# carlostojal/NDT-Net

Hardware: AMD Instinct MI355X
Metric: clouds/sec NDT preprocess+PointNet fwd, 100k pts->1000 NDs, batch=16 (higher is better)
Workload: dtype f64 NDT; PointNet fp32-accurate split-bf16x3 (6 products) on 11 per-point layers, fp32 MFMA on the K=16 first layers and the TNet / seg-bias FC layers

## Files before the change

### include/ndnet_pointnet.h

```cpp
#ifndef NDNET_POINTNET_H_
#define NDNET_POINTNET_H_
#include <stdint.h>

#ifdef __cplusplus
extern "C" {
#endif

#define NDNET_PN_MAX_LAYERS 5

typedef struct ndnet_pn_layer {
  const float* w;
  int64_t w_cloud_stride;
  const float* bias;
  int64_t bias_cloud_stride;
  int32_t K, N;
  int32_t relu;
  int32_t prec;
  int32_t fuse_next;
} ndnet_pn_layer;

typedef struct ndnet_pn_chain {
  const float* x;
  int32_t x_ld;
  int32_t in_cols;
// ... 14 lines not shown
  const float* head_w3;
  const float* head_b3;
  const float* head_basis;
  int32_t head_kin, head_nout;
  float* head_t1;
  const float* fold_t2;
  int32_t fold_ld;
  float* fold_out_w;
  float* fold_out_b;
} ndnet_pn_chain;

int ndnet_pn_chain_run(const ndnet_pn_chain *args, int batch, void *stream);
int ndnet_pn_chain_run_t32(const ndnet_pn_chain *args, int batch, void *stream);

int ndnet_pn_debug_stamps(unsigned long long *host, int wgs);
int ndnet_pn_debug_stamps_clear(void);

int ndnet_pn_fc_run(const float *in, int ld_in, const float *W, const float *bias, float *out, int ld_out,
                    int batch, int K, int N, int relu, void *stream);
int ndnet_pn_fc_mfma_run(const float *in, int ld_in, const float *Wf, const float *bias, float *out, int ld_out,
                         int batch, int K, int N, int relu, void *stream);
int ndnet_pn_cls_head_run(const float *in, int ld_in, const float *Wf, const float *bias, float *probs,
                          int ld_probs, float *logits, int ld_logits, int batch, int K, int N, int out_cols,
                          float *clear, int64_t clear_count, void *stream);
#define NDNET_FOLD_WT 0
#define NDNET_FOLD_FRAG 1
#define NDNET_FOLD_FRAG6 2
#define NDNET_FOLD_ROWS 3
#define NDNET_FOLD_BASIS 4
#define NDNET_FOLD_BIAS 5
typedef struct ndnet_pn_fold_job {
  const float *w;
  const float *bias;
  const float *gamma, *beta, *mean, *var;
  void *out;
  int32_t kind;
  int32_t N, K;
  int32_t ld, k0;
  int32_t Kp, Np;
  int32_t eye;
  float eps;
  int32_t reserved;
  int64_t block0;
} ndnet_pn_fold_job;
int ndnet_pn_fold_prepare(ndnet_pn_fold_job *host_jobs, int num_jobs, int64_t *num_blocks);
int ndnet_pn_fold_run(const ndnet_pn_fold_job *device_jobs, int num_jobs, int64_t num_blocks, void *stream);

int ndnet_pn_head3_run(const float *h2, int ld_h, const float *W3, const float *b3, const float *basis,
                       float *t1, float *w1f, int batch, int K, int kin, int nout, void *stream);

int ndnet_pn_fold_t2_run(const float *w1f, int w1_stride, const float *b1, const float *t2, int t2_ld, float *outf,
                         float *outb, int batch, void *stream);

#ifdef __cplusplus
}
#endif

#endif
```

### ndt-net_amd/csrc/pointnet_kernels.hip

```cpp
#include <hip/hip_runtime.h>
#include <math.h>
#include <stdint.h>
#include <stdio.h>
#include <stdlib.h>

#include "../../include/ndnet_pointnet.h"

namespace {

#ifndef NDNET_PN_TILE
#define NDNET_PN_TILE 64
#endif
constexpr int kP = NDNET_PN_TILE;
#ifndef NDNET_PN_WAVES
#define NDNET_PN_WAVES (NDNET_PN_TILE / 4)
#endif
constexpr int kWaves = NDNET_PN_WAVES;
constexpr int kThreads = 64 * kWaves;
constexpr int kRowBlocks = kP / 16;
static_assert(kP == 64 || kP == 32, "64- or 32-point tiles");
constexpr int kFuseNC = 64;
constexpr int kPadF = 8;
constexpr int kPadB = 16;
#ifndef NDNET_PN_PLANE_SWZ
// ... 1185 lines not shown
#pragma unroll
      for (int b = 0; b < 16; b++) v = lane == b ? acc[b] : v;
      s_part[wave][lane] = v;
    }
    __syncthreads();
    if (wq != 0) return;
    if (lane < 16) {
      float v = 0.0f;
#pragma unroll
      for (int q = 0; q < WPO; q++) v += s_part[wave + q][lane];
      acc[0] = v;
    }
  } else if (lane < 16) {
    float v = 0.0f;
#pragma unroll
    for (int b = 0; b < 16; b++) v = lane == b ? acc[b] : v;
    acc[0] = v;
  }
  if (lane < B && n < N) {
    float v = acc[0] + bias[n];
    if (relu) v = fmaxf(v, 0.0f);
    out[(int64_t)lane * ld_out + n] = v;
  }
}

__global__ void __launch_bounds__(1024) k_pn_fold_t2(const float* __restrict__ w1f, int w1_stride,
                                                     const float* __restrict__ b1, const float* __restrict__ t2,
                                                     int t2_ld, float* __restrict__ outf, float* __restrict__ outb) {
  const int b = blockIdx.x, e = threadIdx.x;
  __shared__ float s_w[13 * 64];
  __shared__ float s_t[64 * 64];
  {
    const float* wb = w1f + (int64_t)b * w1_stride;
    if (e < 16 * 64) {
      const int cb = e >> 8, ln = (e >> 2) & 63, k = 4 * (ln >> 4) + (e & 3), n = 16 * cb + (ln & 15);
      const float v = wb[e];
      if (k < 12) s_w[k * 64 + n] = v;
    }
    if (e < 64) s_w[12 * 64 + e] = b1[e];
    const f32x4* tb = reinterpret_cast<const f32x4*>(t2 + (int64_t)b * t2_ld);
    reinterpret_cast<f32x4*>(s_t)[e] = tb[e];
  }
  __syncthreads();
  if (e < 13 * 64) {
    const int r = e >> 6, n = e & 63;
    float acc = 0.0f;
#pragma unroll 16
    for (int i = 0; i < 64; i++) acc = fmaf(s_w[r * 64 + i], s_t[i * 64 + n], acc);
    if (r < 12) outf[(int64_t)b * 1024 + ((((n >> 4) * 64 + ((r >> 2) & 3) * 16 + (n & 15)) << 2) + (r & 3))] = acc;
    else outb[(int64_t)b * 64 + n] = acc;
  }
}

__global__ void __launch_bounds__(256) k_pn_head3(const float* __restrict__ h2, int ld_h, const float* __restrict__ W3,
                                                  const float* __restrict__ b3, const float* __restrict__ basis,
                                                  float* __restrict__ t1_out, float* __restrict__ w1f, int K, int kin,
                                                  int nout) {
  __shared__ float s_t[9];
  const int b = blockIdx.x;
  const int lane = threadIdx.x & 63, wave = threadIdx.x >> 6;
  const float* h = h2 + (int64_t)b * ld_h;
  for (int o = wave; o < 9; o += 4) {
    float acc = 0.0f;
    for (int k = lane; k < K; k += 64) acc += h[k] * W3[(int64_t)o * K + k];
    for (int off = 32; off > 0; off >>= 1) acc += __shfl_xor(acc, off, 64);
    if (lane == 0) {
      s_t[o] = acc + b3[o];
      t1_out[b * 9 + o] = acc + b3[o];
    }
  }
  const int M = kin * nout, total = 16 * nout;
  auto kn = [&](int e, int& k, int& n) {
    const int cb = e >> 8, ln = (e >> 2) & 63;
    k = 4 * (ln >> 4) + (e & 3);
    n = 16 * cb + (ln & 15);
  };
  constexpr int kE = 4;
  float bas[kE][9];
#pragma unroll
  for (int i = 0; i < kE; i++) {
    const int e = threadIdx.x + i * blockDim.x;
    int k, n;
    kn(e, k, n);
#pragma unroll
    for (int a = 0; a < 9; a++) bas[i][a] = (e < total && k < kin) ? basis[a * M + k * nout + n] : 0.0f;
  }
  __syncthreads();
#pragma unroll
  for (int i = 0; i < kE; i++) {
    const int e = threadIdx.x + i * blockDim.x;
    if (e < total) {
      float acc = 0.0f;
#pragma unroll
      for (int a = 0; a < 9; a++) acc += s_t[a] * bas[i][a];
      w1f[(int64_t)b * total + e] = acc;
    }
  }
  for (int e = threadIdx.x + kE * blockDim.x; e < total; e += blockDim.x) {
    int k, n;
    kn(e, k, n);
    float acc = 0.0f;
    if (k < kin) {
#pragma unroll
      for (int a = 0; a < 9; a++) acc += s_t[a] * basis[a * M + k * nout + n];
    }
    w1f[(int64_t)b * total + e] = acc;
// ... 135 lines not shown
  hipStream_t st = (hipStream_t)stream;
  if (cbw == 4)
    k_pn_fc_mfma<4><<<nb / 4, kFcWaves * 64, 0, st>>>(in, ld_in, wf, bias, out, ld_out, batch, KG, relu);
  else if (cbw == 2)
    k_pn_fc_mfma<2><<<nb / 2, kFcWaves * 64, 0, st>>>(in, ld_in, wf, bias, out, ld_out, batch, KG, relu);
  else
    k_pn_fc_mfma<1><<<nb, kFcWaves * 64, 0, st>>>(in, ld_in, wf, bias, out, ld_out, batch, KG, relu);
  return hipGetLastError() == hipSuccess ? 0 : -21;
}

int ndnet_pn_cls_head_run(const float* in, int ld_in, const float* Wf, const float* bias, float* probs, int ld_probs,
                          float* logits, int ld_logits, int batch, int K, int N, int out_cols, float* clear,
                          int64_t clear_count, void* stream) {
  if (!in || !Wf || !bias || !probs || batch <= 0 || K <= 0 || K % 16 || K > 16 * kClsMaxG || N <= 0 || N % 16 ||
      N > 1024 || out_cols < 1 || out_cols > N || ld_in % 4 || ld_in < K || ld_probs < out_cols ||
      (logits && ld_logits < out_cols) || ((uintptr_t)in | (uintptr_t)Wf) % 16 || clear_count < 0 ||
      (!clear && clear_count))
    return -20;
  k_pn_cls_head<<<(batch + 15) / 16, kClsWaves * 64, (size_t)16 * N * sizeof(float), (hipStream_t)stream>>>(
      in, ld_in, reinterpret_cast<const f32x4*>(Wf), bias, probs, ld_probs, logits, ld_logits, batch, K / 16, N,
      out_cols, clear, clear_count);
  return hipGetLastError() == hipSuccess ? 0 : -21;
}

int ndnet_pn_fc_run(const float* in, int ld_in, const float* W, const float* bias, float* out, int ld_out, int batch,
                    int K, int N, int relu, void* stream) {
  if (!in || !W || !bias || !out || batch <= 0 || batch > 16 || K <= 0 || K % 4 || N <= 0 || ld_in % 4 ||
      ld_in < K || ld_out < N || ((uintptr_t)in | (uintptr_t)W) % 16)
    return -20;
  hipStream_t st = (hipStream_t)stream;
  switch (K % 256 == 0 && K <= 1024 ? K / 256 : 0) {
    case 2: k_pn_fc_split<2><<<(N + 1) / 2, 256, 0, st>>>(in, ld_in, W, bias, out, ld_out, batch, N, relu); break;
    case 4: k_pn_fc_split<4><<<N, 256, 0, st>>>(in, ld_in, W, bias, out, ld_out, batch, N, relu); break;
    default: k_pn_fc<<<(N + 3) / 4, 256, 0, st>>>(in, ld_in, W, bias, out, ld_out, batch, K, N, relu);
  }
  return hipGetLastError() == hipSuccess ? 0 : -21;
}

int ndnet_pn_head3_run(const float* h2, int ld_h, const float* W3, const float* b3, const float* basis, float* t1,
                       float* w1f, int batch, int K, int kin, int nout, void* stream) {
  if (!h2 || !W3 || !b3 || !basis || !t1 || !w1f || batch <= 0 || K <= 0 || ld_h < K || kin <= 0 || kin > 16 ||
      nout <= 0 || nout % 16)
    return -20;
  k_pn_head3<<<batch, 256, 0, (hipStream_t)stream>>>(h2, ld_h, W3, b3, basis, t1, w1f, K, kin, nout);
  return hipGetLastError() == hipSuccess ? 0 : -21;
}

int ndnet_pn_fold_t2_run(const float* w1f, int w1_stride, const float* b1, const float* t2, int t2_ld, float* outf,
                         float* outb, int batch, void* stream) {
  if (!w1f || !b1 || !t2 || !outf || !outb || batch <= 0 || w1_stride < 1024 || t2_ld < 4096 || t2_ld % 4 ||
      (uintptr_t)t2 % 16)
    return -20;
  k_pn_fold_t2<<<batch, 1024, 0, (hipStream_t)stream>>>(w1f, w1_stride, b1, t2, t2_ld, outf, outb);
  return hipGetLastError() == hipSuccess ? 0 : -21;
}

int ndnet_pn_fold_prepare(ndnet_pn_fold_job* jobs, int num_jobs, int64_t* num_blocks) {
  if (!jobs || num_jobs <= 0 || !num_blocks) return -20;
  int64_t blocks = 0;
  for (int i = 0; i < num_jobs; i++) {
    ndnet_pn_fold_job& J = jobs[i];
    const bool bn = J.gamma != nullptr;
    if (!J.out || (uintptr_t)J.out % 16 || J.kind < NDNET_FOLD_WT || J.kind > NDNET_FOLD_BIAS || J.N <= 0 ||
        (bn && (!J.beta || !J.mean || !J.var || !(J.eps >= 0.0f))) || (!bn && (J.beta || J.mean || J.var)))
      return -20;
    if (J.kind == NDNET_FOLD_BIAS) {
      if (!J.bias || J.Np < J.N || J.eye < 0 || (J.eye > 0 && J.eye * J.eye != J.N)) return -20;
    } else {
      if (!J.w || J.K <= 0 || J.k0 < 0 || J.ld < J.k0 + J.K) return -20;
      if (J.kind == NDNET_FOLD_WT && (J.Kp < J.K || J.Np < J.N)) return -20;
      if (J.kind == NDNET_FOLD_FRAG && (J.Kp < J.K || J.Np < J.N || J.Kp % 16 || J.Np % 16)) return -20;
      if (J.kind == NDNET_FOLD_FRAG6 && (J.Kp < J.K || J.Np < J.N || J.Kp % 32 || J.Np % 16)) return -20;
      if (J.kind == NDNET_FOLD_BASIS && J.K != 12) return -20;
    }
    J.block0 = blocks;
    blocks += (fold_units(J) + kFoldThreads - 1) / kFoldThreads;
  }
  if (blocks <= 0 || blocks > 0x7fffffff) return -20;
  *num_blocks = blocks;
  return 0;
}

int ndnet_pn_fold_run(const ndnet_pn_fold_job* jobs, int num_jobs, int64_t num_blocks, void* stream) {
  if (!jobs || num_jobs <= 0 || num_blocks <= 0 || num_blocks > 0x7fffffff) return -20;
  k_pn_fold<<<(unsigned)num_blocks, kFoldThreads, 0, (hipStream_t)stream>>>(jobs, num_jobs);
  return hipGetLastError() == hipSuccess ? 0 : -21;
}


int ndnet_pn_debug_stamps_clear(void) {
#ifdef NDNET_PN_STAMPS
  static unsigned long long zeros[kStampWgs][16];
  return hipMemcpyToSymbol(HIP_SYMBOL(g_pn_stamps), zeros, sizeof(zeros)) == hipSuccess ? 0 : -21;
#else
  return -20;
#endif
}

int ndnet_pn_debug_stamps(unsigned long long* host, int wgs) {
#ifdef NDNET_PN_STAMPS
  if (!host || wgs <= 0 || wgs > kStampWgs) return -20;
  if (hipDeviceSynchronize() != hipSuccess) return -21;
  return hipMemcpyFromSymbol(host, HIP_SYMBOL(g_pn_stamps), (size_t)wgs * 16 * sizeof(unsigned long long)) ==
                 hipSuccess ? 0 : -21;
#else
  (void)host; (void)wgs;
// ... 118 lines not shown
```

### ndt-net_amd/ndnet/_lib.py

```python
from __future__ import annotations

import ctypes
import os

import torch

PKG = os.path.dirname(os.path.abspath(__file__))
ROOT = os.path.dirname(PKG)
LIB_PATH = os.environ.get("NDNET_AMD_LIB") or os.path.join(ROOT, "lib", "libndnet_amd.so")

NDNET_OK = 0
NDNET_ERR_ARG = -20
NDNET_ERR_HIP = -21
NDNET_ERR_SYNC = -22
POINT_FILL = {"none": 0, "nearest": 1}
SEG_CONF_LDS_MAX_COLS = 63
FPS_THREADS = 512
FPS_LDS_POINTS = {"float32": 12288, "float64": 6144}
FPS_REG_POINTS = {"float32": 100352, "float64": 49152}


class NdtStats(ctypes.Structure):
    _fields_ = [
        ("rc", ctypes.c_int32),
# ... 84 lines not shown
    "ndnet_fps_run": (_I, [_P, _I, _U64, _U64, _P, _P, _P, _P, _P]),
    "ndnet_fps_run_f64": (_I, [_P, _I, _U64, _U64, _P, _P, _P, _P, _P]),
    "ndnet_nearest_sample_run": (_I, [_P, _I, _U64, _P, _P, _U64, _P, _P, _P, _P]),
    "ndnet_pn_transform3_run": (_I, [_P, ctypes.c_int64, _P, _P, ctypes.c_int64, _I, _U64, _P]),
    "ndnet_aug_work_bytes": (ctypes.c_size_t, [_I, _U64]),
    "ndnet_aug_run": (_I, [_P, _P, _P, _P, _I, _U64, _P, _P, _P, _P, _P, _P, _P]),
    "ndnet_pts_unpack_i16": (_I, [_P, _P, _I, _U64, _P, _P, _P]),
    "ndnet_ndt_debug_dump": (_I, [_P, _I, _P, _P, _P, _P, _P, _P, _P, _P, _P, _P, _P, _P]),
    "ndnet_ndt_debug_set_epoch": (_I, [_P, ctypes.c_uint32]),
    "ndnet_ndt_debug_set_kl_fuse": (_I, [_P, _I]),
    "ndnet_ndt_debug_set_list_sort": (_I, [_P, _I]),
    "ndnet_ndt_debug_get_list_sort": (_I, [_P]),
    "ndnet_ndt_debug_kl_marks": (_I, [_P, _P]),
    "ndnet_ndt_debug_front_marks": (_I, [_P, _P]),
    "ndnet_ndt_debug_wq_marks": (_I, [_P, _P, ctypes.POINTER(ctypes.c_uint32)]),
    "ndnet_debug_lu_chain": (_I, [_P, ctypes.c_uint32, _I, _P, _P, _P, _P]),
    "ndnet_ndt_debug_front_wg_marks": (_I, [_P, _P, ctypes.POINTER(_I)]),
    "ndnet_ndt_set_timing": (_I, [_P, _I]),
    "ndnet_ndt_stage_ms": (_I, [_P, _P]),
    "ndnet_amd_version": (ctypes.c_char_p, []),
}


def lib() -> ctypes.CDLL:
    global _lib
    if _lib is None:
        if not os.path.exists(LIB_PATH):
            raise RuntimeError(f"{LIB_PATH} is missing: build it with `make -C {ROOT}` "
                               "(there is no CPU fallback)")
        _lib = ctypes.CDLL(LIB_PATH)
        for name, (res, args) in EXPORTS.items():
            fn = getattr(_lib, name)
            fn.restype = res
            fn.argtypes = args
        for name, (res, args) in {**POINTNET_EXPORTS, **TRAIN_EXPORTS}.items():
            fn = getattr(_lib, name)
            fn.restype = res
            fn.argtypes = args
    return _lib


POINTNET_EXPORTS: dict = {
    "ndnet_pn_chain_run": (_I, [_P, _I, _P]),
    "ndnet_pn_chain_run_t32": (_I, [_P, _I, _P]),
    "ndnet_pn_debug_stamps": (_I, [_P, _I]),
    "ndnet_pn_debug_stamps_clear": (_I, []),
    "ndnet_ply_count": (_I, [ctypes.c_char_p, _I, ctypes.POINTER(_U64)]),
    "ndnet_ply_read": (_I, [ctypes.c_char_p, _I, _I, _P, _P, _U64, ctypes.POINTER(_U64), _I]),
    "ndnet_pn_fc_run": (_I, [_P, _I, _P, _P, _P, _I, _I, _I, _I, _I, _P]),
    "ndnet_pn_fc_mfma_run": (_I, [_P, _I, _P, _P, _P, _I, _I, _I, _I, _I, _P]),
    "ndnet_pn_cls_head_run": (_I, [_P, _I, _P, _P, _P, _I, _P, _I, _I, _I, _I, _I, _P, ctypes.c_int64, _P]),
    "ndnet_pn_head3_run": (_I, [_P, _I, _P, _P, _P, _P, _P, _I, _I, _I, _I, _P]),
    "ndnet_pn_fold_t2_run": (_I, [_P, _I, _P, _P, _I, _P, _P, _I, _P]),
    "ndnet_pn_fold_prepare": (_I, [_P, _I, ctypes.POINTER(ctypes.c_int64)]),
    "ndnet_pn_fold_run": (_I, [_P, _I, ctypes.c_int64, _P]),
}


_I64 = ctypes.c_int64

TRAIN_EXPORTS: dict = {
    "ndnet_tr_gemm": (_I, [_P, _P, _P, _P, _I64, _I, _I, _I, _I64, _I64, _I64, _I64, _I64, _I64, _I, _I, _I, _I, _I,
                           _I, _P]),
    "ndnet_tr_sum_parts": (_I, [_P, _P, _I64, _I, _P]),
    "ndnet_tr_sum_parts_2d": (_I, [_P, _P, _I64, _I64, _I64, _I, _P]),
    "ndnet_tr_bn_fwd": (_I, [_P, _P, _P, _P, _P, _P, _P, _P, _I, _I, _I, ctypes.c_float, ctypes.c_float, _I, _P, _P,
                             _P, _P]),
    "ndnet_tr_bn_bwd": (_I, [_P, _P, _P, _P, _P, _P, _P, _P, _P, _P, _I, _I, _I, _I, _P, _P]),
    "ndnet_tr_chan_sum": (_I, [_P, _P, _I, _I, _I, _P]),
    "ndnet_tr_row_sum": (_I, [_P, _P, _I64, _I, _P]),
    "ndnet_tr_argmax_match": (_I, [_P, _P, _I64, _I, _P, _P]),
    "ndnet_tr_argmax_match_cm": (_I, [_P, _P, _I, _I, _I, _P, _P, _P]),
    "ndnet_row_argmax": (_I, [_P, _I64, _I, _P, _P]),
    "ndnet_tr_fc_fwd": (_I, [_P, _P, _P, _P, _P, _P, _P, _P, _P, _P, _P, _I, _I, _I, _I64, ctypes.c_float,
                             ctypes.c_float, _I, _I, _P, _P]),
    "ndnet_tr_fc_bwd_w": (_I, [_P, _P, _P, _P, _P, _P, _P, _P, _P, _P, _P, _P, _I, _I, _I, _I64, _I, _P]),
    "ndnet_tr_fc_bwd_x": (_I, [_P, _P, _P, _P, _I, _I, _I, _I64, _I, _P]),
    "ndnet_tr_point_transform": (_I, [_P, _P, _I, _P, _I, _P, _I, _I, _P]),
    "ndnet_tr_point_transform_bwd": (_I, [_P, _P, _I, _P, _I, _P, _I, _I, _P]),
    "ndnet_tr_log_softmax_c": (_I, [_P, _P, _I, _I, _I, _P]),
    "ndnet_tr_log_softmax_c_bwd": (_I, [_P, _P, _P, _I, _I, _I, _P]),
    "ndnet_tr_nll_onehot": (_I, [_P, _P, _P, _P, _I, _I, _I, _P]),
    "ndnet_tr_nll_onehot_bwd": (_I, [_P, _P, _P, _I, _I, _I, _P]),
    "ndnet_tr_nll_hist": (_I, [_P, _P, _P, _P, _P, _I, _I, _I, _P]),
    "ndnet_tr_nll_hist_bwd": (_I, [_P, _P, _P, _P, _I, _I, _I, _P]),
    "ndnet_tr_hist_match_cm": (_I, [_P, _P, _I, _I, _I, _P, _P, _P]),
    "ndnet_tr_adam": (_I, [_I, _P, _P, _P, _P, _P, _P, _P, ctypes.c_double, ctypes.c_double, ctypes.c_double,
                           ctypes.c_double, _P]),
}


def require_gpu() -> None:
    if not torch.cuda.is_available():
        raise RuntimeError("ndnet_amd needs a ROCm GPU (gfx950); none is visible and there is no CPU fallback")


def check(rc: int, what: str) -> None:
    if rc != NDNET_OK:
        raise RuntimeError(f"{what} failed with code {rc}")


def stream_ptr(device: torch.device | None = None) -> int:
    return torch.cuda.current_stream(device).cuda_stream
```

### ndt-net_amd/ndnet/models/pointnet_hip.py

```python
from __future__ import annotations

import ctypes
import os

import torch

from .. import _lib

MAX_LAYERS = 5
CHAIN_NAMES = ("A: TNet(3) 3-64-128-1024 + max", "B: conv1(t1) + TNet(64) 64-64-128-1024 + max",
               "C: conv1, conv2(t2), conv3 + max", "D: seg head 64-512-256-128-(C+1) + log_softmax")

chain_timing = None

MODES = {"x6": 1, "fp32": 1, "x3": 2, "bf16": 3}
PRECISION = SPLIT_BF16 = X6_PREC = None


def set_precision(mode: str) -> None:
    global PRECISION, SPLIT_BF16, X6_PREC
    if mode not in MODES:
        raise ValueError(f"unknown PointNet precision mode {mode!r}")
    PRECISION = mode
    SPLIT_BF16 = mode != "fp32"
# ... 373 lines not shown
def _use_t32(B: int, n: int, device) -> bool:
    if not TILE32:
        return False
    if device not in _cus:
        _cus[device] = torch.cuda.get_device_properties(device).multi_processor_count
    return 2 * B * ((n + 63) // 64) <= _cus[device]


def _run_chain(ch: "_Chain", x: torch.Tensor, out=None) -> None:
    assert x.stride(1) == ch.x_ld and x.stride(2) == 1 and x.dtype == torch.float32
    ch.x = x.data_ptr()
    ch.out = out.data_ptr() if out is not None else None
    if _use_t32(x.shape[0], x.shape[1], x.device):
        rc = _lib.lib().ndnet_pn_chain_run_t32(ctypes.byref(ch), x.shape[0], _lib.stream_ptr(x.device))
        _lib.check(rc, "ndnet_pn_chain_run_t32")
        return
    rc = _lib.lib().ndnet_pn_chain_run(ctypes.byref(ch), x.shape[0], _lib.stream_ptr(x.device))
    _lib.check(rc, "ndnet_pn_chain_run")


def _chain_torch(x: torch.Tensor, n: int, in_cols: int, layers, relus, mode: int, gmax=None, out=None,
                 out_cols=0, fuse=()) -> None:
    h = x[..., :in_cols].float()
    k0 = layers[0][0].shape[-2]
    h = torch.nn.functional.pad(h, (0, k0 - in_cols))
    for i, (w, b) in enumerate(layers):
        h = torch.matmul(h, w[..., : h.shape[-1], :]) + (b[:, None, :] if b.dim() == 2 else b)
        if relus[i]:
            h = torch.relu(h)
    if mode == 0:
        gmax.copy_(torch.maximum(gmax, h.amax(dim=1)))
    else:
        out.copy_(torch.log_softmax(h[..., :out_cols], dim=2))


class _Workspace:

    def __init__(self, W: _Folded, B: int, N: int, dev, mode: str = None) -> None:
        self.W = W
        self.mode = PRECISION if mode is None else mode
        f32 = dict(dtype=torch.float32, device=dev)
        Fp = W.C_tail[0].shape[1]
        self.gbuf = torch.full((B, 2048 + Fp), float("-inf"), **f32)
        self.g1, self.g2, self.g3 = self.gbuf[:, :1024], self.gbuf[:, 1024:2048], self.gbuf[:, 2048:]
        self.h1, self.h2 = torch.empty((B, 512), **f32), torch.empty((B, 256), **f32)
        self.t1, self.t2 = torch.empty((B, 9), **f32), torch.empty((B, 4096), **f32)
        self.cvec = torch.empty((B, 512), **f32)
        kin = 3 if W.baseline else 12
        self.w1T = None if W.baseline else torch.empty((B, 12, 64), **f32)
        self.w1t2 = torch.empty((B, kin, 64), **f32)
        self.b1t2 = torch.empty((B, 64), **f32)
        self.w1f = None if W.baseline else torch.empty((B, 16 * 64), **f32)
        self.w1t2f = torch.zeros((B, 16 * 64), **f32)
        if W.baseline:
            self.xt = torch.zeros((B, N, 4), **f32)
            self.pts = None
        first = (W.c1T16, W.c1b) if W.baseline else (self.w1T, W.c1b)
        self.specs = [
            (3, W.A, (1, 1, 1), 0, dict(gmax=self.g1)),
            (kin, [first] + W.B_tail, (0, 1, 1, 1), 0, dict(gmax=self.g2)),
            (kin, [(self.w1t2, self.b1t2), W.C_mid, W.C_tail], (0, 0, 0), 0, dict(gmax=self.g3)),
        ]
        if W.seg:
            self.specs.append((kin, [(self.w1t2, self.b1t2), (W.s1aT, self.cvec)] + W.D_tail, (0, 1, 1, 1, 0), 1,
                               dict(out_cols=W.C1, fuse=(1,))))
        self.N = N
        self.structs = {}

    def hip_layers(self, mode: str) -> list:
        W = self.W

        def shared(wb):
            w, b = wb
            if mode != "fp32" and id(w) in W.frag6:
                return (W.frag6[id(w)], 0, b, w.shape[0], w.shape[1], MODES[mode])
            return (W.frag[id(w)], 0, b, w.shape[0], w.shape[1])

        L1 = shared((W.c1T16, W.c1b)) if W.baseline else (self.w1f, self.w1f.stride(0), W.c1b, 16, 64)
        LC = (self.w1t2f, self.w1t2f.stride(0), self.b1t2, 16, 64) if FOLD_T2_KERNEL and not W.baseline else L1
        layers = [
            [shared(x) for x in W.A],
            [L1] + [shared(x) for x in W.B_tail],
            [LC, shared(W.C_mid), shared(W.C_tail)],
        ]
        if W.seg:
            layers.append([(self.w1t2f, self.w1t2f.stride(0), self.b1t2, 16, 64), shared((W.s1aT, self.cvec))] +
                          [shared(x) for x in W.D_tail])
        return layers

    def chain(self, i: int, x: torch.Tensor, chain_fn=None, out=None) -> None:
        in_cols, layers, relus, mode, kw = self.specs[i]
        if chain_fn is not None:
            kw = dict(kw)
            if out is not None:
                kw["out"] = out
            chain_fn(x, self.N, in_cols, layers, relus, mode, **kw)
            return
        structs = self.structs.get(self.mode)
        W = self.W
        if structs is None:
            x_lds = (3, 4, 4, 4) if W.baseline else (12, 12, 12, 12)
            structs = self.structs[self.mode] = [_build_chain(self.N, s[0], hl, s[2], s[3], x_ld=xl, **s[4])
                                                 for s, hl, xl in zip(self.specs, self.hip_layers(self.mode), x_lds)]
            if W.seg:
                structs[3].clear = self.gbuf.data_ptr()
                structs[3].clear_count = self.gbuf.numel()
            if HEAD3_IN_CHAIN and not W.baseline:
                cb = structs[1]
                cb.head_h2, cb.head_ld, cb.head_K = self.h2.data_ptr(), self.h2.stride(0), self.h2.shape[1]
                cb.head_w3, cb.head_b3 = W.t1["f3"].data_ptr(), W.t1["c3"].data_ptr()
                cb.head_basis, cb.head_kin, cb.head_nout = W.t1_basis.data_ptr(), 12, 64
                cb.head_t1 = self.t1.data_ptr()
            if not FOLD_T2_KERNEL or W.baseline:
                cc = structs[2]
                cc.fold_t2, cc.fold_ld = self.t2.data_ptr(), self.t2.stride(0)
                cc.fold_out_w, cc.fold_out_b = self.w1t2f.data_ptr(), self.b1t2.data_ptr()
        if chain_timing is not None:
            e0, e1 = torch.cuda.Event(enable_timing=True), torch.cuda.Event(enable_timing=True)
            e0.record()
            _run_chain(structs[i], x, out)
            e1.record()
            chain_timing.append((i, e0, e1))
        else:
            _run_chain(structs[i], x, out)


def _folded(model):
    cache = model._hip
    if cache is None:
        tensors = _tensors(model)
        cache = model._hip = {"tensors": tensors, "sig": None, "stale": False}
    sig = _signature(cache["tensors"])
    cur = _tensors(model)
    replaced = len(cur) != len(cache["tensors"]) or any(a is not b for a, b in zip(cur, cache["tensors"]))
    if replaced or cache["sig"] != sig or cache["stale"]:
        W = cache.get("W")
        if W is not None and W.can_refold(_tensors(model)):
            W.refold()
        else:
            cache.update(tensors=_tensors(model), W=_Folded(model), ws={})
            sig = _signature(cache["tensors"])
        cache.update(sig=sig, stale=False)
    return cache


FOLD_T2_KERNEL = os.environ.get("NDNET_PN_FOLD_T2", "kernel") == "kernel"
HEAD3_IN_CHAIN = os.environ.get("NDNET_PN_HEAD3", "chain") == "chain"

FC_MFMA = os.environ.get("NDNET_PN_FC", "mfma") == "mfma"


def _fc(x: torch.Tensor, w: torch.Tensor, b: torch.Tensor, out: torch.Tensor, relu: bool, wf=None) -> None:
    B = x.shape[0]
    st = _lib.stream_ptr(x.device)
    for c0 in range(0, B, 16):
        n = min(16, B - c0)
        if FC_MFMA and wf is not None:
            rc = _lib.lib().ndnet_pn_fc_mfma_run(x[c0].data_ptr(), x.stride(0), wf.data_ptr(), b.data_ptr(),
                                                 out[c0].data_ptr(), out.stride(0), n, _pad(w.shape[1], 16),
                                                 w.shape[0], 1 if relu else 0, st)
            _lib.check(rc, "ndnet_pn_fc_mfma_run")
        else:
            rc = _lib.lib().ndnet_pn_fc_run(x[c0].data_ptr(), x.stride(0), w.data_ptr(), b.data_ptr(),
                                            out[c0].data_ptr(), out.stride(0), n, w.shape[1], w.shape[0],
                                            1 if relu else 0, st)
            _lib.check(rc, "ndnet_pn_fc_run")


def _glue_hip(W, ws, B: int):
    st = lambda: _lib.stream_ptr(ws.gbuf.device)

    def fc(x, w, b, out, relu):
        _fc(x, w, b, out, relu, W.fcf.get(id(w)))

    def head_a():
        t = W.t1
        fc(ws.g1, t["f1"], t["c1"], ws.h1, True)
        fc(ws.h1, t["f2"], t["c2"], ws.h2, True)
        if HEAD3_IN_CHAIN:
            return
        for c0 in range(0, B, 16):
            n = min(16, B - c0)
            rc = _lib.lib().ndnet_pn_head3_run(ws.h2[c0].data_ptr(), ws.h2.stride(0), t["f3"].data_ptr(),
                                               t["c3"].data_ptr(), W.t1_basis.data_ptr(), ws.t1[c0].data_ptr(),
                                               ws.w1f[c0].data_ptr(), n, 256, 12, 64, st())
            _lib.check(rc, "ndnet_pn_head3_run")

    def head_a_points():
        t = W.t1
        fc(ws.g1, t["f1"], t["c1"], ws.h1, True)
        fc(ws.h1, t["f2"], t["c2"], ws.h2, True)
        _fc(ws.h2, t["f3"], t["c3"], ws.t1, False, None)
        rc = _lib.lib().ndnet_pn_transform3_run(ws.pts.data_ptr(), ws.pts.stride(1), ws.t1.data_ptr(),
                                                ws.xt.data_ptr(), ws.xt.stride(1), B, ws.pts.shape[1], st())
        _lib.check(rc, "ndnet_pn_transform3_run")

    def head_b():
        t = W.t2
        fc(ws.g2, t["f1"], t["c1"], ws.h1, True)
        fc(ws.h1, t["f2"], t["c2"], ws.h2, True)
        fc(ws.h2, t["f3"], t["c3"], ws.t2, False)
        if FOLD_T2_KERNEL and not W.baseline:
            rc = _lib.lib().ndnet_pn_fold_t2_run(ws.w1f.data_ptr(), ws.w1f.stride(0), W.c1b.data_ptr(),
                                                 ws.t2.data_ptr(), ws.t2.stride(0), ws.w1t2f.data_ptr(),
                                                 ws.b1t2.data_ptr(), B, st())
            _lib.check(rc, "ndnet_pn_fold_t2_run")

    def seg_bias():
        fc(ws.g3[:, : W.F], W.s1g, W.s1b, ws.cvec, False)

    def cls_head(out):
        fc(ws.g3[:, : W.F], W.h1w, W.h1b, ws.h1, True)
        fc(ws.h1, W.h2w, W.h2b, ws.h2, True)
        rc = _lib.lib().ndnet_pn_cls_head_run(ws.h2.data_ptr(), ws.h2.stride(0), W.h3f.data_ptr(), W.h3b.data_ptr(),
                                              out.data_ptr(), out.stride(0), None, 0, B, ws.h2.shape[1], W.Cp, W.C,
                                              ws.gbuf.data_ptr(), ws.gbuf.numel(), st())
        _lib.check(rc, "ndnet_pn_cls_head_run")

    return (head_a_points if W.baseline else head_a), head_b, (seg_bias if W.seg else cls_head)


def _glue_torch(W, ws, B: int):
    def head_a():
        t1 = _fc_head(ws.g1, W.t1, 3, ws.h1, ws.h2, ws.t1)
        torch.matmul(t1.reshape(B, 9), W.t1_basis, out=ws.w1T.view(B, 12 * 64))

    def head_a_points():
        t1 = _fc_head(ws.g1, W.t1, 3, ws.h1, ws.h2, ws.t1)
        ws.xt[..., :3] = torch.nan_to_num(torch.bmm(ws.pts, t1.transpose(1, 2)), nan=0.0)

    def head_b():
        t2 = _fc_head(ws.g2, W.t2, 64, ws.h1, ws.h2, ws.t2)
        torch.matmul(W.c1wT if W.baseline else ws.w1T, t2, out=ws.w1t2)
        torch.matmul(W.c1b[None, None, :], t2, out=ws.b1t2.view(B, 1, 64))

    def seg_bias():
        torch.addmm(W.s1b, ws.g3[:, : W.F], W.s1bT, out=ws.cvec)

    def cls_head(out):
        torch.addmm(W.h1b, ws.g3[:, : W.F], W.h1w[:, :, 0].t(), out=ws.h1).relu_()
        torch.addmm(W.h2b, ws.h1, W.h2w[:, :, 0].t(), out=ws.h2).relu_()
        out.copy_(torch.softmax(torch.addmm(W.h3b[: W.C], ws.h2, W.h3w[:, :, 0].t()), dim=1))

    return (head_a_points if W.baseline else head_a), head_b, (seg_bias if W.seg else cls_head)


_slot = 0


class workspace_slot:

    def __init__(self, slot: int) -> None:
        self.slot, self.prev = int(slot), None

    def __enter__(self):
        global _slot
        self.prev, _slot = _slot, self.slot
        return self

    def __exit__(self, *exc):
        global _slot
        _slot = self.prev
        return False


def _features(model, points: torch.Tensor, covariances: torch.Tensor, chain):
    mode = model_precision(model)
    cache = _folded(model)
    W = cache["W"]
    B, N, _ = points.shape
    dev = points.device
    key = (B, N, dev, _slot)
    ws = cache["ws"].get(key)
    if ws is None:
        ws = cache["ws"][key] = _Workspace(W, B, N, dev, mode)
    ws.mode = mode
    if W.baseline:
        xa = ws.pts = points.float().contiguous()
        x = ws.xt
    elif (points.stride() == (N * 12, 12, 1) and covariances.stride() == (N * 12, 12, 1)
            and covariances.data_ptr() == points.data_ptr() + 12 and points.dtype == torch.float32):
        xa = x = points.as_strided((B, N, 12), (N * 12, 12, 1))
    else:
        xa = x = torch.cat((points, covariances), dim=2).float().contiguous()
    head_a, head_b, last = (_glue_hip if chain is None else _glue_torch)(W, ws, B)
    if chain is not None:
        ws.gbuf.fill_(float("-inf"))
    ws.chain(0, xa, chain)
    head_a()
    ws.chain(1, x, chain)
    head_b()
    ws.chain(2, x, chain)
    return W, ws, x, last


def segmentation_forward(model, points: torch.Tensor, covariances: torch.Tensor, chain=None) -> torch.Tensor:
    W, ws, x, seg_bias = _features(model, points, covariances, chain)
    B, N, _ = points.shape
    seg_bias()
    out = torch.empty((B, N, W.C1), dtype=torch.float32, device=points.device)
    ws.chain(3, x, chain, out=out)
    if chain is not None:
        ws.gbuf.fill_(float("-inf"))
    return out


def classification_forward(model, points: torch.Tensor, covariances: torch.Tensor, chain=None) -> torch.Tensor:
    W, ws, x, cls_head = _features(model, points, covariances, chain)
    out = torch.empty((points.shape[0], W.C), dtype=torch.float32, device=points.device)
    cls_head(out)
    if chain is not None:
        ws.gbuf.fill_(float("-inf"))
    return out.unsqueeze(2)
```

Measured before the change: 89350.

## Collapse linear chain-C layers into one per-cloud 12-to-F affine map

The third PointNet chain (T2-folded conv1, C_mid, C_tail) applies no ReLU between its layers, so the three linear maps are composed per cloud into one 12-input affine layer. A new kernel computes this in double precision on the small weight matrices and writes MFMA-fragment weights and a bias. The per-point chain then runs a single K=16 layer straight into the global max. This removes the large per-point 64x128 and 128xF GEMMs, at the cost of a small per-cloud composition kernel and a change in rounding behaviour.

```diff
diff --git a/include/ndnet_pointnet.h b/include/ndnet_pointnet.h
--- a/include/ndnet_pointnet.h
+++ b/include/ndnet_pointnet.h
@@ -90,6 +90,10 @@
 int ndnet_pn_fold_t2_run(const float *w1f, int w1_stride, const float *b1, const float *t2, int t2_ld, float *outf,
                          float *outb, int batch, void *stream);
 
+int ndnet_pn_fold_collapse_run(const float *w1f, int w1_stride, const float *b1, const float *t2, int t2_ld,
+                               float *outf, float *outb, const float *w2t, const float *b2, const float *w3t,
+                               const float *b3, int F, int Fp, float *mcf, float *ccb, int batch, void *stream);
+
 #ifdef __cplusplus
 }
 #endif
diff --git a/ndt-net_amd/csrc/pointnet_kernels.hip b/ndt-net_amd/csrc/pointnet_kernels.hip
--- a/ndt-net_amd/csrc/pointnet_kernels.hip
+++ b/ndt-net_amd/csrc/pointnet_kernels.hip
@@ -1261,6 +1261,95 @@
   }
 }
 
+constexpr int kCollapseLds = 8 * (128 * 64 + 13 * 64 + 13 * 128) + 4 * (64 * 128 + 64 * 64 + 13 * 64);
+__global__ void __launch_bounds__(1024) k_pn_fold_collapse(const float* __restrict__ w1f, int w1_stride,
+                                                           const float* __restrict__ b1, const float* __restrict__ t2,
+                                                           int t2_ld, float* __restrict__ outf,
+                                                           float* __restrict__ outb, const float* __restrict__ w2t,
+                                                           const float* __restrict__ b2, const float* __restrict__ w3t,
+                                                           const float* __restrict__ b3, int F, int Fp,
+                                                           float* __restrict__ mcf, float* __restrict__ ccb) {
+  const int b = blockIdx.x, e = threadIdx.x;
+  const int r = e >> 6, lane = e & 63;
+  const int n = blockIdx.y * 64 + lane;
+  double* const s_w3 = reinterpret_cast<double*>(g_smem);
+  double* const s_p1 = s_w3 + 128 * 64;
+  double* const s_p2 = s_p1 + 13 * 64;
+  float* const s_w2 = reinterpret_cast<float*>(s_p2 + 13 * 128);
+  float* const s_t = s_w2 + 64 * 128;
+  float* const s_w = s_t + 64 * 64;
+  {
+    const float wv = (w1f + (int64_t)b * w1_stride)[e];
+    const f32x4 tv = reinterpret_cast<const f32x4*>(t2 + (int64_t)b * t2_ld)[e];
+    const f32x4 w2a = reinterpret_cast<const f32x4*>(w2t)[e], w2b = reinterpret_cast<const f32x4*>(w2t)[e + 1024];
+    f32x4 w3v[2];
+#pragma unroll
+    for (int i = 0; i < 2; i++) {
+      const int idx = e + 1024 * i, m = idx >> 4, col = blockIdx.y * 64 + 4 * (idx & 15);
+      w3v[i] = col < Fp ? *reinterpret_cast<const f32x4*>(w3t + (int64_t)m * Fp + col) : f32x4{0.f, 0.f, 0.f, 0.f};
+    }
+    const float b1v = e < 64 ? b1[e] : 0.0f;
+    {
+      const int cb = e >> 8, ln = (e >> 2) & 63, k = 4 * (ln >> 4) + (e & 3), kn = 16 * cb + (ln & 15);
+      if (k < 12) s_w[k * 64 + kn] = wv;
+    }
+    if (e < 64) s_w[12 * 64 + e] = b1v;
+    reinterpret_cast<f32x4*>(s_t)[e] = tv;
+    reinterpret_cast<f32x4*>(s_w2)[e] = w2a;
+    reinterpret_cast<f32x4*>(s_w2)[e + 1024] = w2b;
+#pragma unroll
+    for (int i = 0; i < 2; i++) {
+      double* d = s_w3 + 4 * (e + 1024 * i);
+#pragma unroll
+      for (int q = 0; q < 4; q++) d[q] = (double)w3v[i][q];
+    }
+  }
+  const double b2a = r == 12 ? (double)b2[lane] : 0.0, b2b = r == 12 ? (double)b2[lane + 64] : 0.0;
+  const double b3v = (r == 12 && n < F) ? (double)b3[n] : 0.0;
+  __syncthreads();
+  if (r < 13) {
+    float acc = 0.0f;
+    double acc64 = 0.0;
+#pragma unroll 16
+    for (int i = 0; i < 64; i++) {
+      const float a = s_w[r * 64 + i], t = s_t[i * 64 + lane];
+      acc = fmaf(a, t, acc);
+      acc64 = fma((double)a, (double)t, acc64);
+    }
+    s_p1[r * 64 + lane] = acc64;
+    if (blockIdx.y == 0) {
+      if (r < 12) outf[(int64_t)b * 1024 + ((((lane >> 4) * 64 + ((r >> 2) & 3) * 16 + (lane & 15)) << 2) + (r & 3))] = acc;
+      else outb[(int64_t)b * 64 + lane] = acc;
+    }
+  }
+  __syncthreads();
+  if (r < 13) {
+    double a0 = b2a, a1 = b2b;
+#pragma unroll 16
+    for (int j = 0; j < 64; j++) {
+      const double p = s_p1[r * 64 + j];
+      a0 = fma(p, (double)s_w2[j * 128 + lane], a0);
+      a1 = fma(p, (double)s_w2[j * 128 + lane + 64], a1);
+    }
+    s_p2[r * 128 + lane] = a0;
+    s_p2[r * 128 + lane + 64] = a1;
+  }
+  __syncthreads();
+  if (n >= Fp) return;
+  float v = 0.0f;
+  if (r < 13 && n < F) {
+    double a0 = b3v, a1 = 0.0;
+#pragma unroll 16
+    for (int m = 0; m < 128; m += 2) {
+      a0 = fma(s_p2[r * 128 + m], s_w3[m * 64 + lane], a0);
+      a1 = fma(s_p2[r * 128 + m + 1], s_w3[(m + 1) * 64 + lane], a1);
+    }
+    v = (float)(a0 + a1);
+  }
+  if (r == 12) ccb[(int64_t)b * Fp + n] = v;
+  mcf[(int64_t)b * 16 * Fp + (((n >> 4) * 64 + (r >> 2) * 16 + (n & 15)) << 2) + (r & 3)] = r < 12 ? v : 0.0f;
+}
+
 __global__ void __launch_bounds__(256) k_pn_head3(const float* __restrict__ h2, int ld_h, const float* __restrict__ W3,
                                                   const float* __restrict__ b3, const float* __restrict__ basis,
                                                   float* __restrict__ t1_out, float* __restrict__ w1f, int K, int kin,
@@ -1502,6 +1591,26 @@
       (uintptr_t)t2 % 16)
     return -20;
   k_pn_fold_t2<<<batch, 1024, 0, (hipStream_t)stream>>>(w1f, w1_stride, b1, t2, t2_ld, outf, outb);
+  return hipGetLastError() == hipSuccess ? 0 : -21;
+}
+
+int ndnet_pn_fold_collapse_run(const float* w1f, int w1_stride, const float* b1, const float* t2, int t2_ld,
+                               float* outf, float* outb, const float* w2t, const float* b2, const float* w3t,
+                               const float* b3, int F, int Fp, float* mcf, float* ccb, int batch, void* stream) {
+  if (!w1f || !b1 || !t2 || !outf || !outb || batch <= 0 || w1_stride < 1024 || t2_ld < 4096 || t2_ld % 4 ||
+      (uintptr_t)t2 % 16)
+    return -20;
+  if (!w2t || !b2 || !w3t || !b3 || !mcf || !ccb || F < 1 || Fp < F || Fp % 16) return -20;
+  if (((uintptr_t)w2t | (uintptr_t)w3t) % 16) return -20;
+  static bool attr_set = false;
+  if (!attr_set) {
+    if (hipFuncSetAttribute((const void*)k_pn_fold_collapse, hipFuncAttributeMaxDynamicSharedMemorySize,
+                            kCollapseLds) != hipSuccess)
+      return -21;
+    attr_set = true;
+  }
+  k_pn_fold_collapse<<<dim3(batch, (Fp + 63) / 64), 1024, kCollapseLds, (hipStream_t)stream>>>(
+      w1f, w1_stride, b1, t2, t2_ld, outf, outb, w2t, b2, w3t, b3, F, Fp, mcf, ccb);
   return hipGetLastError() == hipSuccess ? 0 : -21;
 }
 
diff --git a/ndt-net_amd/ndnet/_lib.py b/ndt-net_amd/ndnet/_lib.py
--- a/ndt-net_amd/ndnet/_lib.py
+++ b/ndt-net_amd/ndnet/_lib.py
@@ -160,6 +160,7 @@
     "ndnet_pn_cls_head_run": (_I, [_P, _I, _P, _P, _P, _I, _P, _I, _I, _I, _I, _I, _P, ctypes.c_int64, _P]),
     "ndnet_pn_head3_run": (_I, [_P, _I, _P, _P, _P, _P, _P, _I, _I, _I, _I, _P]),
     "ndnet_pn_fold_t2_run": (_I, [_P, _I, _P, _P, _I, _P, _P, _I, _P]),
+    "ndnet_pn_fold_collapse_run": (_I, [_P, _I, _P, _P, _I, _P, _P, _P, _P, _P, _P, _I, _I, _P, _P, _I, _P]),
     "ndnet_pn_fold_prepare": (_I, [_P, _I, ctypes.POINTER(ctypes.c_int64)]),
     "ndnet_pn_fold_run": (_I, [_P, _I, ctypes.c_int64, _P]),
 }
diff --git a/ndt-net_amd/ndnet/models/pointnet_hip.py b/ndt-net_amd/ndnet/models/pointnet_hip.py
--- a/ndt-net_amd/ndnet/models/pointnet_hip.py
+++ b/ndt-net_amd/ndnet/models/pointnet_hip.py
@@ -452,11 +452,19 @@
         if W.baseline:
             self.xt = torch.zeros((B, N, 4), **f32)
             self.pts = None
+        self.collapse = collapse_applies(W)
+        if self.collapse:
+            self.mcT = torch.zeros((B, 12, Fp), **f32)
+            self.mcf = torch.zeros((B, 16 * Fp), **f32)
+            self.cc = torch.zeros((B, Fp), **f32)
+            chain_c = (kin, [(self.mcT, self.cc)], (0,), 0, dict(gmax=self.g3))
+        else:
+            chain_c = (kin, [(self.w1t2, self.b1t2), W.C_mid, W.C_tail], (0, 0, 0), 0, dict(gmax=self.g3))
         first = (W.c1T16, W.c1b) if W.baseline else (self.w1T, W.c1b)
         self.specs = [
             (3, W.A, (1, 1, 1), 0, dict(gmax=self.g1)),
             (kin, [first] + W.B_tail, (0, 1, 1, 1), 0, dict(gmax=self.g2)),
-            (kin, [(self.w1t2, self.b1t2), W.C_mid, W.C_tail], (0, 0, 0), 0, dict(gmax=self.g3)),
+            chain_c,
         ]
         if W.seg:
             self.specs.append((kin, [(self.w1t2, self.b1t2), (W.s1aT, self.cvec)] + W.D_tail, (0, 1, 1, 1, 0), 1,
@@ -475,10 +483,14 @@
 
         L1 = shared((W.c1T16, W.c1b)) if W.baseline else (self.w1f, self.w1f.stride(0), W.c1b, 16, 64)
         LC = (self.w1t2f, self.w1t2f.stride(0), self.b1t2, 16, 64) if FOLD_T2_KERNEL and not W.baseline else L1
+        if self.collapse:
+            chain_c = [(self.mcf, self.mcf.stride(0), self.cc, 16, self.cc.shape[1])]
+        else:
+            chain_c = [LC, shared(W.C_mid), shared(W.C_tail)]
         layers = [
             [shared(x) for x in W.A],
             [L1] + [shared(x) for x in W.B_tail],
-            [LC, shared(W.C_mid), shared(W.C_tail)],
+            chain_c,
         ]
         if W.seg:
             layers.append([(self.w1t2f, self.w1t2f.stride(0), self.b1t2, 16, 64), shared((W.s1aT, self.cvec))] +
@@ -542,6 +554,13 @@
 
 
 FOLD_T2_KERNEL = os.environ.get("NDNET_PN_FOLD_T2", "kernel") == "kernel"
+COLLAPSE = os.environ.get("NDNET_PN_COLLAPSE", "1") == "1"
+
+
+def collapse_applies(W) -> bool:
+    return bool(COLLAPSE) and FOLD_T2_KERNEL and not W.baseline
+
+
 HEAD3_IN_CHAIN = os.environ.get("NDNET_PN_HEAD3", "chain") == "chain"
 
 FC_MFMA = os.environ.get("NDNET_PN_FC", "mfma") == "mfma"
@@ -597,7 +616,14 @@
         fc(ws.g2, t["f1"], t["c1"], ws.h1, True)
         fc(ws.h1, t["f2"], t["c2"], ws.h2, True)
         fc(ws.h2, t["f3"], t["c3"], ws.t2, False)
-        if FOLD_T2_KERNEL and not W.baseline:
+        if ws.collapse:
+            Fp = ws.cc.shape[1]
+            rc = _lib.lib().ndnet_pn_fold_collapse_run(
+                ws.w1f.data_ptr(), ws.w1f.stride(0), W.c1b.data_ptr(), ws.t2.data_ptr(), ws.t2.stride(0),
+                ws.w1t2f.data_ptr(), ws.b1t2.data_ptr(), W.C_mid[0].data_ptr(), W.C_mid[1].data_ptr(),
+                W.C_tail[0].data_ptr(), W.C_tail[1].data_ptr(), W.F, Fp, ws.mcf.data_ptr(), ws.cc.data_ptr(), B, st())
+            _lib.check(rc, "ndnet_pn_fold_collapse_run")
+        elif FOLD_T2_KERNEL and not W.baseline:
             rc = _lib.lib().ndnet_pn_fold_t2_run(ws.w1f.data_ptr(), ws.w1f.stride(0), W.c1b.data_ptr(),
                                                  ws.t2.data_ptr(), ws.t2.stride(0), ws.w1t2f.data_ptr(),
                                                  ws.b1t2.data_ptr(), B, st())
@@ -617,6 +643,17 @@
     return (head_a_points if W.baseline else head_a), head_b, (seg_bias if W.seg else cls_head)
 
 
+def compose_chain_c(w1T: torch.Tensor, b1: torch.Tensor, t2: torch.Tensor, mid, tail):
+    B = w1T.shape[0]
+    p = torch.cat((w1T.double(), b1.double().expand(B, 1, 64)), dim=1)
+    p = torch.matmul(p, t2.double())
+    for wT, b in (mid, tail):
+        p = torch.matmul(p, wT.double())
+        p[:, 12, : b.shape[0]] += b.double()
+    p = p.float()
+    return p[:, :12], p[:, 12]
+
+
 def _glue_torch(W, ws, B: int):
     def head_a():
         t1 = _fc_head(ws.g1, W.t1, 3, ws.h1, ws.h2, ws.t1)
@@ -630,6 +667,10 @@
         t2 = _fc_head(ws.g2, W.t2, 64, ws.h1, ws.h2, ws.t2)
         torch.matmul(W.c1wT if W.baseline else ws.w1T, t2, out=ws.w1t2)
         torch.matmul(W.c1b[None, None, :], t2, out=ws.b1t2.view(B, 1, 64))
+        if ws.collapse:
+            mc, cc = compose_chain_c(ws.w1T, W.c1b, t2, W.C_mid, W.C_tail)
+            ws.mcT.copy_(mc)
+            ws.cc.copy_(cc)
 
     def seg_bias():
         torch.addmm(W.s1b, ws.g3[:, : W.F], W.s1bT, out=ws.cvec)
@@ -667,7 +708,7 @@
     W = cache["W"]
     B, N, _ = points.shape
     dev = points.device
-    key = (B, N, dev, _slot)
+    key = (B, N, dev, _slot) if collapse_applies(W) else (B, N, dev, _slot, "layered")
     ws = cache["ws"].get(key)
     if ws is None:
         ws = cache["ws"][key] = _Workspace(W, B, N, dev, mode)
```

After: 88470. No clear change (-1.0%).

## Collapse linear C-chain layers into one per-cloud folded weight matrix

Applied to the files above, without the earlier changes.

Adds a kernel that, after the feature-transform fold, multiplies the per-cloud 12x64 first-layer weights (plus bias row) through the C_mid (64->128) and C_tail (128->Fp) weights with fp32 MFMA. The product is a single per-cloud K=16 weight and bias. The point-wise chain C then runs one layer instead of three, removing two wide per-point GEMMs over every point. This relies on the intermediate C layers having no nonlinearity, and it changes rounding because the products are precombined in fp32 rather than evaluated per point with split-bf16. It also adds a small per-cloud precompute grid and larger per-cloud weight buffers.

```diff
diff --git a/include/ndnet_pointnet.h b/include/ndnet_pointnet.h
--- a/include/ndnet_pointnet.h
+++ b/include/ndnet_pointnet.h
@@ -90,6 +90,10 @@
 int ndnet_pn_fold_t2_run(const float *w1f, int w1_stride, const float *b1, const float *t2, int t2_ld, float *outf,
                          float *outb, int batch, void *stream);
 
+int ndnet_pn_fold_t2_collapse_run(const float *w1f, int w1_stride, const float *b1, const float *t2, int t2_ld,
+                                  const float *w2t, const float *b2, const float *w3t, const float *b3, int Fp,
+                                  float *outf, float *outb, float *wcf, float *bc, int batch, void *stream);
+
 #ifdef __cplusplus
 }
 #endif
diff --git a/ndt-net_amd/csrc/pointnet_kernels.hip b/ndt-net_amd/csrc/pointnet_kernels.hip
--- a/ndt-net_amd/csrc/pointnet_kernels.hip
+++ b/ndt-net_amd/csrc/pointnet_kernels.hip
@@ -1261,6 +1261,96 @@
   }
 }
 
+#if NDNET_PN_TILE == 64
+constexpr int kColP1 = 64 + kPadF, kColP2 = 128 + kPadF;
+__global__ void __launch_bounds__(1024) k_pn_fold_t2_collapse(
+    const float* __restrict__ w1f, int w1_stride, const float* __restrict__ b1, const float* __restrict__ t2, int t2_ld,
+    const float* __restrict__ w2t, const float* __restrict__ b2, const float* __restrict__ w3t,
+    const float* __restrict__ b3, int Fp, float* __restrict__ outf, float* __restrict__ outb, float* __restrict__ wcf,
+    float* __restrict__ bc) {
+  const int b = blockIdx.y, e = threadIdx.x;
+  const int lane = e & 63, wave = e >> 6;
+  const int fr = lane & 15, fk = lane >> 4;
+  const int n0 = blockIdx.x * 64;
+  __shared__ float s_w[13 * 64];
+  __shared__ __attribute__((aligned(16))) float s_t[64 * 64];
+  __shared__ __attribute__((aligned(16))) float s_u[16 * kColP1];
+  __shared__ __attribute__((aligned(16))) float s_v[16 * kColP2];
+  {
+    const float* wb = w1f + (int64_t)b * w1_stride;
+    {
+      const int cb = e >> 8, ln = (e >> 2) & 63, k = 4 * (ln >> 4) + (e & 3), n = 16 * cb + (ln & 15);
+      const float v = wb[e];
+      if (k < 12) s_w[k * 64 + n] = v;
+    }
+    if (e < 64) s_w[12 * 64 + e] = b1[e];
+    const f32x4* tb = reinterpret_cast<const f32x4*>(t2 + (int64_t)b * t2_ld);
+    reinterpret_cast<f32x4*>(s_t)[e] = tb[e];
+  }
+  float w2r[16], w3r[32];
+  float bias2 = 0.0f, bias3 = 0.0f;
+  const bool tail = wave < 4 && n0 + 16 * wave < Fp;
+  if (wave >= 8) {
+    const float* p = w2t + 16 * (wave - 8) + fr;
+#pragma unroll
+    for (int i = 0; i < 16; i++) w2r[i] = p[(16 * (i >> 2) + 4 * fk + (i & 3)) * 128];
+    if (fk == 3) bias2 = b2[16 * (wave - 8) + fr];
+  } else if (tail) {
+    const float* p = w3t + n0 + 16 * wave + fr;
+#pragma unroll
+    for (int i = 0; i < 32; i++) w3r[i] = p[(int64_t)(16 * (i >> 2) + 4 * fk + (i & 3)) * Fp];
+    if (fk == 3) bias3 = b3[n0 + 16 * wave + fr];
+  }
+  __syncthreads();
+  {
+    const int r = e >> 6, n = e & 63;
+    float acc = 0.0f;
+    if (e < 13 * 64) {
+#pragma unroll 16
+      for (int i = 0; i < 64; i++) acc = fmaf(s_w[r * 64 + i], s_t[i * 64 + n], acc);
+      if (blockIdx.x == 0) {
+        if (r < 12) outf[(int64_t)b * 1024 + ((((n >> 4) * 64 + ((r >> 2) & 3) * 16 + (n & 15)) << 2) + (r & 3))] = acc;
+        else outb[(int64_t)b * 64 + n] = acc;
+      }
+    }
+    s_u[r * kColP1 + n] = acc;
+  }
+  __syncthreads();
+  if (wave >= 8) {
+    f32x4 v = {bias2, 0.f, 0.f, 0.f};
+#pragma unroll
+    for (int g = 0; g < 4; g++) {
+      const f32x4 a = *reinterpret_cast<const f32x4*>(s_u + fr * kColP1 + 16 * g + 4 * fk);
+#pragma unroll
+      for (int s = 0; s < 4; s++) v = __builtin_amdgcn_mfma_f32_16x16x4f32(a[s], w2r[4 * g + s], v, 0, 0, 0);
+    }
+#pragma unroll
+    for (int r = 0; r < 4; r++) s_v[(4 * fk + r) * kColP2 + 16 * (wave - 8) + fr] = v[r];
+  }
+  __syncthreads();
+  if (tail) {
+    f32x4 v0 = {bias3, 0.f, 0.f, 0.f}, v1 = {0.f, 0.f, 0.f, 0.f};
+#pragma unroll
+    for (int g = 0; g < 8; g += 2) {
+      const f32x4 a0 = *reinterpret_cast<const f32x4*>(s_v + fr * kColP2 + 16 * g + 4 * fk);
+      const f32x4 a1 = *reinterpret_cast<const f32x4*>(s_v + fr * kColP2 + 16 * (g + 1) + 4 * fk);
+#pragma unroll
+      for (int s = 0; s < 4; s++) {
+        v0 = __builtin_amdgcn_mfma_f32_16x16x4f32(a0[s], w3r[4 * g + s], v0, 0, 0, 0);
+        v1 = __builtin_amdgcn_mfma_f32_16x16x4f32(a1[s], w3r[4 * (g + 1) + s], v1, 0, 0, 0);
+      }
+    }
+    f32x4 v = v0 + v1;
+    const int n = n0 + 16 * wave + fr;
+    if (fk == 3) {
+      bc[(int64_t)b * Fp + n] = v[0];
+      v = f32x4{0.f, 0.f, 0.f, 0.f};
+    }
+    reinterpret_cast<f32x4*>(wcf + (int64_t)b * 16 * Fp)[(n >> 4) * 64 + lane] = v;
+  }
+}
+#endif
+
 __global__ void __launch_bounds__(256) k_pn_head3(const float* __restrict__ h2, int ld_h, const float* __restrict__ W3,
                                                   const float* __restrict__ b3, const float* __restrict__ basis,
                                                   float* __restrict__ t1_out, float* __restrict__ w1f, int K, int kin,
@@ -1502,6 +1592,18 @@
       (uintptr_t)t2 % 16)
     return -20;
   k_pn_fold_t2<<<batch, 1024, 0, (hipStream_t)stream>>>(w1f, w1_stride, b1, t2, t2_ld, outf, outb);
+  return hipGetLastError() == hipSuccess ? 0 : -21;
+}
+
+int ndnet_pn_fold_t2_collapse_run(const float* w1f, int w1_stride, const float* b1, const float* t2, int t2_ld,
+                                  const float* w2t, const float* b2, const float* w3t, const float* b3, int Fp,
+                                  float* outf, float* outb, float* wcf, float* bc, int batch, void* stream) {
+  if (!w1f || !b1 || !t2 || !w2t || !b2 || !w3t || !b3 || !outf || !outb || !wcf || !bc || batch <= 0 ||
+      batch > 65535 || w1_stride < 1024 || t2_ld < 4096 || t2_ld % 4 || Fp <= 0 || Fp % 16 ||
+      ((uintptr_t)t2 | (uintptr_t)wcf) % 16)
+    return -20;
+  k_pn_fold_t2_collapse<<<dim3((Fp + 63) / 64, batch), 1024, 0, (hipStream_t)stream>>>(
+      w1f, w1_stride, b1, t2, t2_ld, w2t, b2, w3t, b3, Fp, outf, outb, wcf, bc);
   return hipGetLastError() == hipSuccess ? 0 : -21;
 }
 
diff --git a/ndt-net_amd/ndnet/_lib.py b/ndt-net_amd/ndnet/_lib.py
--- a/ndt-net_amd/ndnet/_lib.py
+++ b/ndt-net_amd/ndnet/_lib.py
@@ -160,6 +160,7 @@
     "ndnet_pn_cls_head_run": (_I, [_P, _I, _P, _P, _P, _I, _P, _I, _I, _I, _I, _I, _P, ctypes.c_int64, _P]),
     "ndnet_pn_head3_run": (_I, [_P, _I, _P, _P, _P, _P, _P, _I, _I, _I, _I, _P]),
     "ndnet_pn_fold_t2_run": (_I, [_P, _I, _P, _P, _I, _P, _P, _I, _P]),
+    "ndnet_pn_fold_t2_collapse_run": (_I, [_P, _I, _P, _P, _I, _P, _P, _P, _P, _I, _P, _P, _P, _P, _I, _P]),
     "ndnet_pn_fold_prepare": (_I, [_P, _I, ctypes.POINTER(ctypes.c_int64)]),
     "ndnet_pn_fold_run": (_I, [_P, _I, ctypes.c_int64, _P]),
 }
diff --git a/ndt-net_amd/ndnet/models/pointnet_hip.py b/ndt-net_amd/ndnet/models/pointnet_hip.py
--- a/ndt-net_amd/ndnet/models/pointnet_hip.py
+++ b/ndt-net_amd/ndnet/models/pointnet_hip.py
@@ -449,6 +449,8 @@
         self.b1t2 = torch.empty((B, 64), **f32)
         self.w1f = None if W.baseline else torch.empty((B, 16 * 64), **f32)
         self.w1t2f = torch.zeros((B, 16 * 64), **f32)
+        self.wCf = torch.zeros((B, 16 * Fp), **f32)
+        self.bC = torch.zeros((B, Fp), **f32)
         if W.baseline:
             self.xt = torch.zeros((B, N, 4), **f32)
             self.pts = None
@@ -475,10 +477,14 @@
 
         L1 = shared((W.c1T16, W.c1b)) if W.baseline else (self.w1f, self.w1f.stride(0), W.c1b, 16, 64)
         LC = (self.w1t2f, self.w1t2f.stride(0), self.b1t2, 16, 64) if FOLD_T2_KERNEL and not W.baseline else L1
+        if collapse_c(W, mode):
+            chain_c = [(self.wCf, self.wCf.stride(0), self.bC, 16, self.bC.shape[1])]
+        else:
+            chain_c = [LC, shared(W.C_mid), shared(W.C_tail)]
         layers = [
             [shared(x) for x in W.A],
             [L1] + [shared(x) for x in W.B_tail],
-            [LC, shared(W.C_mid), shared(W.C_tail)],
+            chain_c,
         ]
         if W.seg:
             layers.append([(self.w1t2f, self.w1t2f.stride(0), self.b1t2, 16, 64), shared((W.s1aT, self.cvec))] +
@@ -542,6 +548,13 @@
 
 
 FOLD_T2_KERNEL = os.environ.get("NDNET_PN_FOLD_T2", "kernel") == "kernel"
+COLLAPSE_C = os.environ.get("NDNET_PN_COLLAPSE_C", "1") != "0"
+
+
+def collapse_c(W, mode: str) -> bool:
+    return COLLAPSE_C and FOLD_T2_KERNEL and not W.baseline and mode in ("x6", "fp32")
+
+
 HEAD3_IN_CHAIN = os.environ.get("NDNET_PN_HEAD3", "chain") == "chain"
 
 FC_MFMA = os.environ.get("NDNET_PN_FC", "mfma") == "mfma"
@@ -597,7 +610,13 @@
         fc(ws.g2, t["f1"], t["c1"], ws.h1, True)
         fc(ws.h1, t["f2"], t["c2"], ws.h2, True)
         fc(ws.h2, t["f3"], t["c3"], ws.t2, False)
-        if FOLD_T2_KERNEL and not W.baseline:
+        if collapse_c(W, ws.mode):
+            rc = _lib.lib().ndnet_pn_fold_t2_collapse_run(
+                ws.w1f.data_ptr(), ws.w1f.stride(0), W.c1b.data_ptr(), ws.t2.data_ptr(), ws.t2.stride(0),
+                W.C_mid[0].data_ptr(), W.C_mid[1].data_ptr(), W.C_tail[0].data_ptr(), W.C_tail[1].data_ptr(),
+                ws.bC.shape[1], ws.w1t2f.data_ptr(), ws.b1t2.data_ptr(), ws.wCf.data_ptr(), ws.bC.data_ptr(), B, st())
+            _lib.check(rc, "ndnet_pn_fold_t2_collapse_run")
+        elif FOLD_T2_KERNEL and not W.baseline:
             rc = _lib.lib().ndnet_pn_fold_t2_run(ws.w1f.data_ptr(), ws.w1f.stride(0), W.c1b.data_ptr(),
                                                  ws.t2.data_ptr(), ws.t2.stride(0), ws.w1t2f.data_ptr(),
                                                  ws.b1t2.data_ptr(), B, st())
```

New measurement: 88370 before, 88770 after (median of 6 runs). Within noise of the previous version (+0.4%).
